# jweyn/DLWP-CS

Hardware: AMD Instinct MI355X
Metric: cubed-sphere samples/sec (fwd+bwd) (higher is better)
Workload: dtype bf16; 1 GPU; unet2 C48: x (32,6,48,48,14) per GPU, 14 out channels, base 32, MSE + Adam, fwd+bwd+update, bf16 activations + bf16 MFMA, fp32 master weights / gradients / Adam; global_batch=32, parallelism=dp1, hip_graphs=True

## Files before the change

dlwp-cs_amd/DLWP/_native.py:

```python
import ctypes
import os
import threading

import numpy as np
import torch

_HERE = os.path.dirname(os.path.abspath(__file__))
_TAG = os.environ.get('DLWPCS_LIB_TAG', '')
LIB_PATH = os.path.join(os.path.dirname(_HERE), 'lib', 'libdlwpcs%s.so' % ('_' + _TAG if _TAG else ''))

F32 = 0
BF16 = 1
MSE_TARGET_F32 = 0x100
MSE_OVERWRITE = 0x200
ADAM_ZERO_GRAD = 1
HEAD_DEFER_STAGE2 = 2
LOSS_MSE, LOSS_MAE, LOSS_ACC = 0, 1, 2
REG_NONE, REG_MSE, REG_MAE, REG_GLOBAL = 0, 1, 2, 3
ACT_NONE = 0
ACT_LEAKY_CLIP = 1
CONV_ACCUMULATE_WGRAD = 1
CONV_PREPACKED = 2
CONV_REUSE_DZ = 4
CONV_DEFER_REDUCE = 8
# ... 118 lines not shown
    'dlwpcs_wgrad_batch_apply': (c_int, [c_void_p, c_int, c_void_p, c_void_p, c_void_p, c_void_p, c_void_p, c_void_p, c_size_t,
                                         c_void_p, c_void_p, c_void_p, c_void_p, c_void_p]),
    'dlwpcs_gconv_fwd': (c_int, [ctypes.POINTER(GConvDesc)] + [c_void_p] * 9),
    'dlwpcs_gconv_bwd_data': (c_int, [ctypes.POINTER(GConvDesc)] + [c_void_p] * 6),
    'dlwpcs_gconv_bwd_weights': (c_int, [ctypes.POINTER(GConvDesc)] + [c_void_p] * 9),
    'dlwpcs_act_fwd': (c_int, [c_void_p, c_void_p, c_size_t, c_int, c_float, c_float, c_int, c_void_p]),
    'dlwpcs_act_bwd': (c_int, [c_void_p, c_void_p, c_void_p, c_size_t, c_int, c_float, c_float, c_int, c_void_p]),
    'dlwpcs_avgpool2_fwd': (c_int, [c_void_p, c_void_p, c_int, c_int, c_int, c_int, c_void_p]),
    'dlwpcs_avgpool2_bwd': (c_int, [c_void_p, c_void_p, c_int, c_int, c_int, c_int, c_void_p]),
    'dlwpcs_avgpool2_bwd_add': (c_int, [c_void_p, c_void_p, c_void_p, c_int, c_int, c_int, c_int, c_void_p]),
    'dlwpcs_avgpool2_bwd_masked': (c_int, [c_void_p, c_void_p, c_void_p, c_void_p, c_int, c_int, c_int, c_float, c_float, c_int,
                                           c_void_p]),
    'dlwpcs_avgpool2_bwd_ring': (c_int, [c_void_p, c_void_p, c_void_p, c_void_p, c_int, c_int, c_int, c_float, c_float, c_int,
                                         c_void_p, c_void_p, c_int, c_int, c_void_p]),
    'dlwpcs_conv_ring_info': (c_int, [ctypes.POINTER(ConvDesc), ctypes.POINTER(c_size_t), ctypes.POINTER(c_int)]),
    'dlwpcs_upsample2_fwd': (c_int, [c_void_p, c_void_p, c_int, c_int, c_int, c_int, c_void_p]),
    'dlwpcs_upsample2_bwd': (c_int, [c_void_p, c_void_p, c_int, c_int, c_int, c_int, c_void_p]),
    'dlwpcs_concat2': (c_int, [c_void_p, c_void_p, c_void_p, c_size_t, c_int, c_int, c_int, c_void_p]),
    'dlwpcs_split2': (c_int, [c_void_p, c_void_p, c_void_p, c_size_t, c_int, c_int, c_int, c_void_p]),
    'dlwpcs_cf_to_cl': (c_int, [c_void_p, c_void_p, c_int, c_int, c_size_t, c_int, c_void_p]),
    'dlwpcs_cl_to_cf': (c_int, [c_void_p, c_void_p, c_int, c_int, c_size_t, c_int, c_void_p]),
    'dlwpcs_add': (c_int, [c_void_p, c_void_p, c_void_p, c_size_t, c_int, c_void_p]),
    'dlwpcs_l1l2_regularize': (c_int, [c_void_p, c_void_p, c_size_t, c_float, c_float, c_float, c_void_p, c_void_p]),
    'dlwpcs_weight_constraint': (c_int, [c_void_p, c_int, c_int, c_int, c_float, c_float, c_float, c_void_p]),
    'dlwpcs_mse_scratch_bytes': (c_size_t, []),
    'dlwpcs_mse_fwd_bwd': (c_int, [c_void_p, c_void_p, c_void_p, c_void_p, c_size_t, c_float, c_int, c_void_p,
                                   c_void_p]),
    'dlwpcs_loss_scratch_bytes': (c_size_t, []),
    'dlwpcs_loss_fwd_bwd': (c_int, [c_void_p, c_void_p, c_void_p, c_void_p, c_void_p, c_size_t, c_int, c_void_p, c_void_p]),
    'dlwpcs_head_loss_step': (c_int, [c_void_p, c_void_p, c_void_p, c_void_p, c_void_p, c_void_p, c_void_p, c_void_p, c_void_p,
# ... 26 lines not shown
    'dlwpcs_batch_gather': (c_int, [c_void_p, ctypes.c_int64, c_int, ctypes.c_int64, c_void_p, c_int, c_void_p, c_int,
                                    c_int, c_int, c_int, c_void_p, c_int, c_int, c_int, c_int, c_int, c_void_p]),
    'dlwpcs_solar_fill': (c_int, [c_void_p, ctypes.c_int64, c_void_p, ctypes.c_int64, c_void_p, c_int, c_int, c_int, c_int,
                                  c_void_p, c_int, c_int, c_int, c_int, c_int, c_void_p]),
    'dlwpcs_comm_load': (c_int, [ctypes.c_char_p]),
    'dlwpcs_comm_unique_id': (c_int, [c_void_p]),
    'dlwpcs_comm_init': (c_int, [ctypes.POINTER(c_void_p), c_void_p, c_int, c_int]),
    'dlwpcs_comm_destroy': (c_int, [c_void_p]),
    'dlwpcs_allreduce_f32': (c_int, [c_void_p, c_void_p, c_size_t, c_void_p]),
    'dlwpcs_lds_oob_probe': (c_int, [c_void_p, c_void_p]),
    'dlwpcs_prof_enable': (c_int, [c_int]),
    'dlwpcs_prof_reset': (c_int, []),
    'dlwpcs_prof_count': (c_int, []),
    'dlwpcs_prof_get': (c_int, [c_int, ctypes.c_char_p, c_int, ctypes.POINTER(ctypes.c_double),
                                ctypes.POINTER(ctypes.c_double), ctypes.POINTER(ctypes.c_double)]),
    'dlwpcs_prof_known_tags': (c_int, []),
    'dlwpcs_prof_known_tag': (c_int, [c_int, ctypes.c_char_p, c_int]),
}

_lib = None
_lock = threading.Lock()


class NativeError(RuntimeError):
    pass


def lib():
    global _lib
    if _lib is None:
# ... 130 lines not shown
```

dlwp-cs_amd/csrc/common.h:

```cpp
#pragma once
#include <hip/hip_runtime.h>
#include <stdint.h>
#include <stdio.h>
#include <stdarg.h>
#include <string.h>
#include "../../include/dlwpcs.h"

namespace dlwpcs {

void set_error(const char *fmt, ...);
int fail(int code, const char *fmt, ...);
const char *last_error();

inline int check_launch(const char *what) {
    hipError_t e = hipGetLastError();
    if (e != hipSuccess) return fail(DLWPCS_E_LAUNCH, "%s: %s", what, hipGetErrorString(e));
    return DLWPCS_OK;
}

bool prof_enabled();
int prof_begin(const char *tag, double flops, double bytes, hipStream_t s);
void prof_end(int idx, hipStream_t s);
int prof_register_tag(const char *tag);
template <typename T> struct KTagType { static const char *str() { return nullptr; } };
template <> struct KTagType<float> { static const char *str() { return "float"; } };
template <> struct KTagType<unsigned short> { static const char *str() { return "unsigned short"; } };
template <typename Name, typename T, auto... Vs> struct KTag {
    static void fmt(char *&p, char *end, bool v) { p += snprintf(p, end - p, "%s", v ? "true" : "false"); }
    static void fmt(char *&p, char *end, int v) { p += snprintf(p, end - p, "%d", v); }
    static const char *str() {
        static char buf[200];
        if (!buf[0]) {
            char *p = buf, *end = buf + sizeof(buf);
            p += snprintf(p, end - p, "%s<", Name::str());
            bool first = true;
            if (KTagType<T>::str()) { p += snprintf(p, end - p, "%s", KTagType<T>::str()); first = false; }
            ((p += snprintf(p, end - p, "%s", first ? "" : ", "), fmt(p, end, Vs), first = false), ...);
// ... 141 lines not shown
```

dlwp-cs_amd/csrc/conv_launch.h:

```cpp
#pragma once
#include "conv_ws.h"

namespace dlwpcs {

struct Work { double flops, bytes; };

static int tile_pixels(int BM, int No) {
    const int face_pix = No * No;
    int pix = BM < face_pix ? BM : face_pix;
    if (No <= BM) {
        int whole = (BM / No) * No;
        if (whole > face_pix) whole = face_pix;
        if (ceil_div(face_pix, whole) <= ceil_div(face_pix, pix)) pix = whole;
    }
    return pix;
}

static long ilv_cost(int pix, int face_pix, int B, int gx, int WM, int *gb, int *fb, bool split, int c2 = 2) {
    auto cost = [&](int npix) { const int mn = (npix + 31) / 32; return 4 * ceil_div(mn, WM) + c2; };
    const int nbl = ceil_div(face_pix, pix), cF = cost(pix), cL = cost(face_pix - (nbl - 1) * pix);
    const long ntiles = 6l * B * nbl;
    const long plain = (long)ceil_div((int)ntiles, gx) * cF;
    if (gb) *gb = 0;
    if (fb) *fb = 0;
    if (!split || cL >= cF || nbl < 2) return plain;
    const long F = 6l * (nbl - 1) * B, S = 6l * B;
    long best = plain;
    for (int GB = 1; GB < gx; ++GB) {
        const int GA = gx - GB;
        const long sB = ceil_div((int)S, GB) * (long)cL;
        for (long mB = 0; mB <= ceil_div((int)F, gx) + 1; ++mB) {
            const long FB = mB * GB < F ? mB * GB : F, FA = F - FB;
            const long cA = (long)ceil_div((int)FA, GA) * cF, cB = mB * cF + sB;
            const long mx = cA > cB ? cA : cB;
            if (mx < best) { best = mx; if (gb) *gb = GB; if (fb) *fb = (int)FB; }
        }
    }
    return best;
}

extern thread_local ConvEdgeArgs g_edge_args;

struct ConvWsName { static const char *str() { return "conv_mfma_ws_kernel"; } };

template <typename T, int KS, int KC, int MT, int NT, int WM, int WN, int VW, int MODE, bool MASK, bool TAIL8 = false, bool MOUT = false,
          bool EDGE = false>
static int launch_conv_cfg(ConvKParams P, const Work &W, hipStream_t s) {
    constexpr int ES = sizeof(T), CGW = 32 / ES;
    constexpr int BM = 32 * MT * WM, NTB = NT * WN, NTHREADS = 64 * WM * WN;
    const int face_pix = P.No * P.No;
    P.ncol = 1;
    if (MODE == MODE_HALO && !EDGE && KS == 3 && (tune_bits() & TUNE_CONV_STRIPS) && P.No >= 64 && P.No % 2 == 0 && P.Cout % (16 / ES) == 0) {
        const int wt = P.No / 2, rows2 = BM / wt, rows1 = BM / P.No;
        if (BM % wt == 0 && rows2 <= P.No && P.No % rows2 == 0 && rows1 >= 1 && rows2 >= 2 * rows1) P.ncol = 2;
    }
    P.Wt = P.No / P.ncol;
// ... 35 lines not shown
    bool pool = MODE != MODE_ZERO && P.pool_out != nullptr && P.No % 2 == 0 && P.Wt % 2 == 0 && (rowpairs || halfrows) &&
                strip_pix % pix == 0 && P.Cout % 32 == 0 && P.Cout % (16 / ES) == 0;
    if (EDGE) pool = pool && !MOUT && ES == 2 && P.dsplit > 0 && P.dsplit % 32 == 0;
    const size_t buf = in_b + w_b;
    size_t patch_b = (size_t)(WM * WN) * 32 * (32 * ES + 16);
    if (pool && 2 * buf + patch_b * MT <= 160 * 1024) patch_b *= MT; else pool = false;
    size_t lds = 2 * buf + patch_b;
    P.patches = 1;
    P.wstat = 0;
    const int nchunks = ceil_div(P.CG, KC / CGW);
    if (nchunks > 2 && nchunks <= 4 && (tune_bits() & TUNE_CONV_WSTAT) && 2 * in_b + nchunks * w_b + patch_b <= 160 * 1024) {
        P.wstat = nchunks;
        lds = 2 * in_b + nchunks * w_b + patch_b;
    } else if (lds > 160 * 1024) { lds = 2 * buf; P.patches = 0; pool = false; }
    if (!pool) P.pool_out = nullptr;
    {
        const bool head = P.head_w != nullptr && P.head_out != nullptr && ES == 2 && NT == 1 && WN == 1 && !EDGE && !MOUT && !MASK &&
                          MODE != MODE_ZERO && P.Cout == 32 && P.patches && !pool;
        if (head) P.out = P.head_out; else P.head_w = nullptr;
        if (P.head_done) *P.head_done = head ? 1 : 0;
    }
    P.colsplit = (pool && halfrows) ? 1 : 0;
    if (P.pool_done) *P.pool_done = pool ? 1 : 0;
    if ((MODE == MODE_ZERO || EDGE) && KS == 3 && P.patches && P.Cout % (16 / ES) == 0 && P.dsplit % (16 / ES) == 0) {
        if (P.direct_done) *P.direct_done = (P.d0 || P.d1) ? 1 : 0;
    } else {
        P.d0 = P.d1 = nullptr;
    }
    if (EDGE) {
        if (P.nblk_face < 2)
// ... 7 lines not shown
        return fail(DLWPCS_E_UNSUPPORTED, "conv: %d tile rows exceed the producers' 5-bit row field", P.tile_rows_max);
    if ((size_t)P.tile_rows_max * P.W2 > (size_t)3 * NTHREADS)
        return fail(DLWPCS_E_UNSUPPORTED, "conv: tile of %d x %d pixels exceeds the producers' register capacity", P.tile_rows_max, P.W2);
    if ((long)6 * face_pix * P.Cout * ES >= (1l << 31))
        return fail(DLWPCS_E_UNSUPPORTED, "conv: one sample of the output (%ld bytes) exceeds the 32-bit store offsets",
                    (long)6 * face_pix * P.Cout * ES);
    if ((long)P.Nin * P.Nin * 6 >= (1l << 16) * 6 && (long)P.Nin * P.Nin >= (1l << 16))
        return fail(DLWPCS_E_UNSUPPORTED, "conv: face size %d too large for the 16-bit index arithmetic", P.Nin);
    auto kern = conv_mfma_ws_kernel<T, KS, KC, MT, NT, WM, WN, VW, MODE, MASK, TAIL8, MOUT, EDGE>;
    if (!MOUT || !(P.d0 || P.d1)) {
        if (!(P.d0)) P.m0 = nullptr;
        if (!(P.d1)) P.m1 = nullptr;
        if (!MOUT) P.m0 = P.m1 = nullptr;
    }
    if (P.mask_done) *P.mask_done = (MOUT && (P.m0 || P.m1)) ? ((P.m0 ? 1 : 0) | (P.m1 ? 2 : 0)) : 0;
    if (lds > 64 * 1024) {
        hipError_t e = hipFuncSetAttribute((const void *)kern, hipFuncAttributeMaxDynamicSharedMemorySize, (int)lds);
        if (e != hipSuccess) return fail(DLWPCS_E_LAUNCH, "conv: hipFuncSetAttribute: %s", hipGetErrorString(e));
    }
    const int gy = ceil_div(P.NTtot, NTB);
    int gx = 256 / gy;
    if (gx < 1) gx = 1;
    if (gx > P.ntiles) gx = P.ntiles;
    dim3 grid((unsigned)gx, (unsigned)gy);
    if (MODE == MODE_ZERO && MT == 3 && sizeof(T) == 4 && (P.tune & TUNE_CONV_ILV) && P.nblk_face > 1 && gx > 1)
        (void)ilv_cost(pix, face_pix, P.B, gx, WM, &P.split_gb, &P.split_fb, true);
    if (P.ilv_fwd) { P.split_gb = fwd_gb; P.split_fb = fwd_fb; }
    if (P.dry_run) return DLWPCS_OK;
    int pidx = -1;
    const char *tag = KTag<ConvWsName, T, KS, KC, MT, NT, WM, WN, VW, MODE, MASK, TAIL8, MOUT, EDGE>::tag();
    if (prof_enabled()) {
        pidx = prof_begin(tag, W.flops, W.bytes, s);
    }
    hipLaunchKernelGGL(kern, grid, dim3(2 * NTHREADS), lds, s, P, g_edge_args);
    if (pidx >= 0) prof_end(pidx, s);
    return check_launch("conv_mfma");
}

template <typename T, int KS, int VW, int MODE, bool MASK, bool MOUT = false, bool EDGE = false>
static int launch_conv(const ConvKParams &P, const Work &W, hipStream_t s) {
    const int face_pix = P.No * P.No;
    constexpr int VWF = 16 / (int)sizeof(T);
    constexpr int K2 = 64 / (int)sizeof(T);
    constexpr int K1 = K2 / 2;
    if constexpr (KS == 1) return launch_conv_cfg<T, KS, K1, 3, 1, 4, 1, VW, MODE, MASK, false, MOUT, EDGE>(P, W, s);
    else if constexpr (VW != VWF) return launch_conv_cfg<T, KS, K1, 3, 1, 4, 1, VW, MODE, MASK, false, MOUT, EDGE>(P, W, s);
    else {
// ... 35 lines not shown
```

dlwp-cs_amd/csrc/conv_mfma.hip:

```cpp
#include <stdlib.h>
#include <type_traits>
#include "common.h"
#include "mfma_common.h"
#include "conv_ws.h"
#include "conv_launch.h"

namespace dlwpcs {

template <typename T>
__device__ __forceinline__ void pack_weights_range(const float *__restrict__ w_eq, const float *__restrict__ w_pol,
                                                   const float *__restrict__ w_np, T *__restrict__ out,
                                                   int KS, int Cin, int Cout, int K, int Ncol, int CG, int NTtot,
                                                   int flip, int transposed, size_t total, size_t first, size_t stride) {
    constexpr int J = 16 / (int)sizeof(T);
    const int TAPS = KS * KS;
    const size_t entries = total / J;
    for (size_t e = first; e < entries; e += stride) {
        unsigned r = (unsigned)e;
        const int n = r % 32; r /= 32;
        const int hf = r % 2; r /= 2;
        const int tap = r % TAPS; r /= TAPS;
        const int cg = r % CG; r /= CG;
        const int nt = r % NTtot; r /= NTtot;
        const int v = (int)r;
// ... 1108 lines not shown
}

static bool pw_applies(const dlwpcs_conv_desc *d) {
    return d->dtype == DLWPCS_BF16 && d->ksize == 1 && !d->halo && !d->up0 && d->C1 == 0 && d->C0 == 32 && d->Cout % 2 == 0 &&
           d->Cout >= 8 && d->Cout <= 32 && ((long)d->N * d->N) % 16 == 0 && d->B > 0 &&
           (long)d->B * 6 * d->N * d->N * 32 < (1l << 31);
}
static unsigned pw_grid(long ngroups) {
    long blocks = (ngroups + 4 * PW_U - 1) / (4 * PW_U);
    return (unsigned)(blocks > 2048 ? 2048 : blocks);
}

static inline int cin_logical(const dlwpcs_conv_desc *d);

thread_local ConvEdgeArgs g_edge_args{};

struct WgradBf16Name { static const char *str() { return "wgrad_bf16_kernel"; } };
struct WgradMfmaName { static const char *str() { return "wgrad_mfma_kernel"; } };
struct PwHeadName { static const char *str() { return "pw_head_train_kernel"; } };
struct PwFwdName { static const char *str() { return "pw_fwd_kernel"; } };
static const int g_plain_tags[] = {prof_register_tag("pw_dgrad_kernel<false>"), prof_register_tag("pw_dgrad_kernel<true>"),
                                   prof_register_tag("wgrad_reduce_batch_kernel")};

static int dispatch_conv(int dtype, int KS, int vw, const ConvKParams &P, const Work &W, hipStream_t s) {
    if (KS == 3 && P.mode == MODE_HALO && P.edge) {
        if (dtype == DLWPCS_BF16 && vw == 8) return dispatch_conv_edge(P, W, s);
        return fail(DLWPCS_E_UNSUPPORTED, "conv: gather-form data gradient serves bf16 with 16-B channel vectors");
    }
    return dtype == DLWPCS_BF16 ? dispatch_conv_bf16(KS, vw, P, W, s) : dispatch_conv_f32(KS, vw, P, W, s);
}
// ... 390 lines not shown
    const int NTtot = ceil_div(d->Cout, 32);
    if (b_eq && !prepacked) {
        const int n = 3 * NTtot * 32;
        hipLaunchKernelGGL(pack_bias_kernel, dim3(ceil_div(n, 256)), dim3(256), 0, s, (const float *)b_eq,
                           (const float *)b_pol, (const float *)b_np, (float *)(ws + L.bias), d->Cout, NTtot * 32);
    }
    ConvKParams P{};
    P.src0 = src0; P.src1 = src1; P.ymask = nullptr;
    P.wpk = wpk; P.bias = b_eq ? bpk : nullptr; P.out = y; P.table = table_dev;
    P.B = d->B; P.Nin = d->N; P.No = out_size(d);
    P.C0 = d->C0; P.C1 = d->C1; P.Cin = Cin; P.Cout = d->Cout;
    P.CG = ceil_div(Cin, cgw_of(d->dtype)); P.NTtot = NTtot; P.up0 = d->up0;
    P.mode = d->halo ? MODE_HALO : MODE_DIRECT;
    P.act = d->act; P.alpha = d->alpha; P.vmax = d->vmax;
    P.pool_out = y_pooled; P.pool_done = pool_done;
    if (head) { P.head_w = head->wpk; P.head_b = head->bias; P.head_out = head->out; P.head_done = head->done; }
    if ((d->flags & DLWPCS_CONV_OUT_PADDED) && !pw_applies(d))
        return fail(DLWPCS_E_UNSUPPORTED, "conv_fwd: DLWPCS_CONV_OUT_PADDED serves the bf16 pointwise output layer only");
    if (pw_applies(d)) {
        PwParams Q{};
        Q.in = (const bf16_t *)src0; Q.wpk = (const bf16_t *)wpk; Q.bias = b_eq ? bpk : nullptr; Q.out = (bf16_t *)y;
        Q.ngroups = (long)d->B * 6 * d->N * d->N / 16; Q.groups_per_face = d->N * d->N / 16; Q.Cout = d->Cout;
        if (d->flags & DLWPCS_CONV_OUT_PADDED) Q.Cout = (d->Cout + 7) / 8 * 8;
        Q.alpha = d->alpha; Q.vmax = d->vmax;
        int pidx = -1;
        const bool actv = d->act != DLWPCS_ACT_NONE;
        if (prof_enabled()) {
            const Work wk = conv_work(d);
            const char *tag = Q.Cout <= 16 ? (actv ? KTag<PwFwdName, void, true, 1>::tag() : KTag<PwFwdName, void, false, 1>::tag())
                                           : (actv ? KTag<PwFwdName, void, true, 2>::tag() : KTag<PwFwdName, void, false, 2>::tag());
// ... 4 lines not shown
            if (actv) hipLaunchKernelGGL((pw_fwd_kernel<true, 1>), pgrid, dim3(256), 0, s, Q);
            else hipLaunchKernelGGL((pw_fwd_kernel<false, 1>), pgrid, dim3(256), 0, s, Q);
        } else {
            if (actv) hipLaunchKernelGGL((pw_fwd_kernel<true, 2>), pgrid, dim3(256), 0, s, Q);
            else hipLaunchKernelGGL((pw_fwd_kernel<false, 2>), pgrid, dim3(256), 0, s, Q);
        }
        if (pidx >= 0) prof_end(pidx, s);
        return check_launch("pw_fwd");
    }
    if (d->dtype == DLWPCS_BF16 && d->ksize == 3 && d->halo && d->C1 == 0 && d->C0 >= 8 && d->C0 % 2 == 0 && d->C0 % 8 != 0 &&
        NTtot <= 2) {
        return dispatch_conv_tail8(d->C0 <= 16 ? 16 : 32, NTtot, P, conv_work(d), s);
    }
    return dispatch_conv(d->dtype, d->ksize, vec_width(d->C0, d->C1, d->dtype), P, conv_work(d), s);
}

static int conv_bwd_data_impl(const dlwpcs_conv_desc *d, const void *dy, const void *y, bool dz_given,
                              const void *w_eq, const void *w_pol, const void *w_np,
                              void *dsrc0, void *dsrc1, const void *m0, const void *m1, float m_alpha, float m_vmax,
                              const int32_t *inv_table_dev, void *workspace, size_t workspace_bytes, dlwpcs_stream_t stream,
                              const char *who, int *ring_query = nullptr) {
    int rc = validate(d, who);
    if (rc) return rc;
    const bool prepacked = (d->flags & DLWPCS_CONV_PREPACKED) != 0;
    if (!dy || !w_eq || (!w_pol && !prepacked) || !workspace) return fail(DLWPCS_E_INVALID, "%s: null pointer", who);
    const bool has_act = d->act != DLWPCS_ACT_NONE && !dz_given;
    if (has_act && !y) return fail(DLWPCS_E_INVALID, "%s: activation needs the saved output y", who);
    if (d->halo && !inv_table_dev) return fail(DLWPCS_E_INVALID, "%s: halo requested without inverse table", who);
    if ((m0 || m1) && (!(m_alpha >= 0.f) || !(m_vmax >= 0.f)))
        return fail(DLWPCS_E_INVALID, "%s: mask activation needs negative_slope >= 0 and max_value >= 0, got %g / %g", who, m_alpha, m_vmax);
// ... 162 lines not shown
    if (!d->halo || d->ksize != 3 || d->up0 || d->B < 1) return 0;
    const WsLayout L = ws_layout(d);
    int q = 0;
    char dummy = 0;
    dlwpcs_conv_desc dd = *d;
    dd.act = DLWPCS_ACT_NONE;
    dd.flags |= DLWPCS_CONV_PREPACKED;
    const int rc = conv_bwd_data_impl(&dd, &dummy, nullptr, true, &dummy, nullptr, nullptr, &dummy, d->C1 > 0 ? &dummy : nullptr, nullptr,
                                      nullptr, 0.f, 0.f, (const int32_t *)&dummy, &dummy, L.total, nullptr, "conv_ring_info", &q);
    if (rc || !q) return 0;
    *dxv_offset = L.dxv;
    *channels = d->C0 + d->C1;
    return 1;
}

extern "C" int dlwpcs_conv_bwd_weights(const dlwpcs_conv_desc *d, const void *src0, const void *src1, const void *dy,
                                       const void *y, void *dw_eq, void *dw_pol, void *dw_np,
                                       void *db_eq, void *db_pol, void *db_np, const int32_t *table_dev,
                                       void *workspace, size_t workspace_bytes, dlwpcs_stream_t stream) {
    int rc = validate(d, "conv_bwd_weights");
    if (rc) return rc;
    if (!src0 || !dy || !dw_eq || !dw_pol || !workspace) return fail(DLWPCS_E_INVALID, "conv_bwd_weights: null pointer");
    if (d->C1 > 0 && !src1) return fail(DLWPCS_E_INVALID, "conv_bwd_weights: C1 > 0 but src1 is null");
    if (d->act != DLWPCS_ACT_NONE && !y) return fail(DLWPCS_E_INVALID, "conv_bwd_weights: activation needs the saved output y");
    if (d->halo && !table_dev) return fail(DLWPCS_E_INVALID, "conv_bwd_weights: halo requested without table");
    if ((db_np != nullptr) != (dw_np != nullptr) && db_eq) return fail(DLWPCS_E_INVALID, "conv_bwd_weights: dw_np/db_np must match");
    const WsLayout L = ws_layout(d);
    if (workspace_bytes < L.total) return fail(DLWPCS_E_WORKSPACE, "conv_bwd_weights: workspace %zu < %zu bytes", workspace_bytes, L.total);
    hipStream_t s = (hipStream_t)stream;
    char *ws = (char *)workspace;
// ... 195 lines not shown
```

dlwp-cs_amd/csrc/conv_ws.h:

```cpp
#pragma once
#include <stdlib.h>
#include <type_traits>
#include "common.h"
#include "mfma_common.h"

namespace dlwpcs {

enum { MODE_DIRECT = 0, MODE_HALO = 1, MODE_ZERO = 2 };

struct ConvKParams {
    const void *src0, *src1;
    const void *ymask;
    const void *wpk;
    const float *bias;
    void *out;
    const int32_t *table;
    int edge;
    int B, Nin, No;
    int C0, C1, Cin, Cout;
    int CG, NTtot;
    int up0;
    int mode;
    int act;
    float alpha, vmax;
// ... 21 lines not shown
    void *head_out;
    int *head_done;
    int tune;
    int tile_rows_max;
    int ntiles;
    int split_gb, split_fb;
    int Wt, ncol;
    uint32_t magicWt, magicNcol;
    int ilv_fwd;
};

struct ConvEdgeArgs { const int32_t *src; int8_t wids[36]; };

enum { TUNE_WG_PRODUCER_PRIO = 1, TUNE_CONV_PRODUCER_PRIO = 2, TUNE_CONV_WEIGHTS_STAY = 4, TUNE_CONV_SPLIT_N = 16,
       TUNE_CONV_SPLIT2_BWD = 32, TUNE_CONV_WSTAT = 64, TUNE_CONV_STAGGER = 256, TUNE_CONV_ILV = 512, TUNE_CONV_STRIPS = 1024,
       TUNE_CONV_ILV_FWD = 2048 };
static int tune_bits() {
    static int v = -1;
    if (v < 0) { const char *e = getenv("DLWPCS_TUNE"); v = e ? atoi(e) : (TUNE_WG_PRODUCER_PRIO | TUNE_CONV_PRODUCER_PRIO | TUNE_CONV_WEIGHTS_STAY | TUNE_CONV_SPLIT_N | TUNE_CONV_SPLIT2_BWD | TUNE_CONV_WSTAT |
                               TUNE_CONV_STAGGER | TUNE_CONV_ILV | TUNE_CONV_STRIPS | TUNE_CONV_ILV_FWD | (3 << 12));
                 }
    return v;
}

template <typename T, int KS, int KC, int MT, int NT, int WM, int WN, int VW, int MODE, bool MASK, bool TAIL8 = false, bool MOUT = false,
          bool EDGE = false>
__device__ __forceinline__ void conv_ws_body(const ConvKParams &P, char *smem, const uint32_t lw, const int G, const int by,
                                             const ConvEdgeArgs &E = ConvEdgeArgs{}) {
    static_assert(!TAIL8 || (VW == 8 && sizeof(T) == 2 && !MASK), "TAIL8: bf16 16-B vectors, forward only");
    static_assert(!MOUT || ((MODE == MODE_ZERO || EDGE) && KS == 3 && sizeof(T) == 2 && !MASK), "MOUT: bf16 data gradient, direct mode");
    static_assert(!EDGE || (MODE == MODE_HALO && KS == 3 && !MASK && !TAIL8 && VW * sizeof(T) == 16), "EDGE: gather-form data gradient");
// ... 18 lines not shown
    typedef typename VecT<T, VW>::type V;
    const int in_bytes = P.tile_rows_max * P.W2 * RB;
    const int in_step = P.wstat ? in_bytes : in_bytes + WF4 * 16;
    const int w_base = P.wstat ? 2 * in_bytes : in_bytes;
    const int w_step = P.wstat ? WF4 * 16 : in_bytes + WF4 * 16;
    const int patch_base = P.wstat ? 2 * in_bytes + P.wstat * WF4 * 16 : 2 * (in_bytes + WF4 * 16);

    const int tid = threadIdx.x;
    const bool is_producer = tid >= NCT;
    const int nt0 = by * NTB;
    const int face_pix = P.No * P.No;
    const int strip_pix = P.No * P.Wt;
    const int g0 = P.up0 ? (P.Nin >> 1) : P.Nin;
    const int nchunks = (P.CG + KCG - 1) / KCG;

    constexpr bool ILV_OK = (MODE == MODE_ZERO || (MODE == MODE_HALO && !EDGE && KS == 3)) && MT == 3 && sizeof(T) == 4;
    const bool ilv = ILV_OK && (P.tune & TUNE_CONV_ILV) != 0 && (MODE == MODE_ZERO || P.ilv_fwd != 0);
    const int nbl = P.nblk_face;
    const bool csplit = ilv && P.split_gb > 0;
    int t_first = 0, t_last = 0;
    int f0 = 0, f1 = 0, s0 = 0, s1 = 0;
    if (csplit) {
        const int GB = P.split_gb, GA = G - GB;
        const int Ftot = 6 * (nbl - 1) * P.B, Stot = 6 * P.B, FA = Ftot - P.split_fb;
        if ((int)lw < GA) {
            f0 = (int)(((long)FA * lw) / GA); f1 = (int)(((long)FA * (lw + 1)) / GA);
        } else {
            const int u = (int)lw - GA;
            f0 = FA + (int)(((long)P.split_fb * u) / GB); f1 = FA + (int)(((long)P.split_fb * (u + 1)) / GB);
            s0 = (int)(((long)Stot * u) / GB); s1 = (int)(((long)Stot * (u + 1)) / GB);
        }
    } else {
        t_first = (int)(((long)P.ntiles * lw) / G);
        t_last = (int)(((long)P.ntiles * (lw + 1)) / G);
    }
    const int n_my = csplit ? (f1 - f0) + (s1 - s0) : t_last - t_first;
    auto tile_of = [&](int q) __attribute__((always_inline)) {
        if (!csplit) return t_first + q;
        const int nf = f1 - f0, perF = (nbl - 1) * P.B;
        if (q < nf) { const int i = f0 + q, f = i / perF; return f * nbl * P.B + (i - f * perF); }
        const int i = s0 + (q - nf), f = i / P.B;
        return f * nbl * P.B + perF + (i - f * P.B);
    };
    if ((P.tune & TUNE_CONV_STAGGER) && !csplit && n_my * G < P.ntiles) {
#pragma unroll 1
// ... 670 lines not shown
        load_frag(0, fa[0], fb[0]);
        __builtin_amdgcn_sched_group_barrier(0x100, MTA + NT, 0);
#pragma unroll
        for (int step = 0; step < NSTEP; ++step) {
            const int cur = step & 1;
            if (step + 1 < NSTEP) load_frag(step + 1, fa[cur ^ 1], fb[cur ^ 1]);
#pragma unroll
            for (int mt = 0; mt < MTA; ++mt)
#pragma unroll
                for (int nt = 0; nt < NT; ++nt) frag_mma<T>(acc[mt][nt], fb[cur][nt], fa[cur][mt]);
            __builtin_amdgcn_sched_group_barrier(0x100, MTA + NT, 0);
            __builtin_amdgcn_sched_group_barrier(0x008, MmaPerFrag<T>::N * MTA * NT, 0);
        }
    };

    auto mma_chunk_edge = [&](const Geo &gq, int ch, auto two_tag) {
      if constexpr (EDGE) {
        constexpr int NSETS = decltype(two_tag)::value ? 2 : 1;
        constexpr int NX = NSETS * 3 * KCG;
        const char *lds_in = smem + (g & 1) * in_step, *lds_w = smem + w_base + (P.wstat ? ch : (g & 1)) * w_step;
        const char *lds_x = lds_w + WF4M * 16;
        uint32_t (&rs)[MT][3] = es;
        uint32_t (&rw)[(MT + 3) / 4] = ewp;
#pragma unroll
        for (int mt = 0; mt < MT; ++mt) asm volatile("" : "+v"(rs[mt][0]), "+v"(rs[mt][1]), "+v"(rs[mt][2]));
#pragma unroll
        for (int w = 0; w < (MT + 3) / 4; ++w) asm volatile("" : "+v"(rw[w]));
        uint4 fa[2][MT], fb[2][NT];
        auto load_frag = [&](int step, uint4 (&a)[MT], uint4 (&bw)[NT]) {
            if (step < NSTEP) {
                const int cgl = step / TAPS, tap = step % TAPS;
                const int dy = tap / KS, dx = tap % KS;
                const int tapoff = (dy * P.W2 + dx) * RB + cgl * 32;
#pragma unroll
                for (int mt = 0; mt < MT; ++mt) {
                    int base = abase[mt];
                    if (tap != TAPS / 2) base += (int)((rw[mt / 4] >> (8 * (mt % 4) + (tap < TAPS / 2 ? tap : tap - 1))) & 1u) << 23;
                    a[mt] = *reinterpret_cast<const uint4 *>(lds_in + base + tapoff);
                }
#pragma unroll
                for (int nt = 0; nt < NT; ++nt)
                    bw[nt] = *reinterpret_cast<const uint4 *>(
                        lds_w + ((((wn * NT + nt) * KCG + cgl) * TAPS + tap) * 2 + half) * 512 + l31 * 16);
            } else {
                const int x = step - NSTEP, j = x / KCG, cgl = x % KCG;
#pragma unroll
                for (int mt = 0; mt < MT; ++mt) {
                    const uint32_t f16 = (j & 1) ? rs[mt][j >> 1] >> 16 : rs[mt][j >> 1] & 0xffffu;
                    a[mt] = *reinterpret_cast<const uint4 *>(lds_in + (int)(f16 << 4) + cgl * 32);
                }
#pragma unroll
                for (int nt = 0; nt < NT; ++nt)
                    bw[nt] = *reinterpret_cast<const uint4 *>(
                        lds_x + (((j % 3) * NTB * KCG + (wn * NT + nt) * KCG + cgl) * 2 + half) * 512 + l31 * 16);
            }
        };
        load_frag(0, fa[0], fb[0]);
        __builtin_amdgcn_sched_group_barrier(0x100, MT + NT, 0);
#pragma unroll
        for (int step = 0; step < NSTEP + NX; ++step) {
            const int cur = step & 1;
            if (step + 1 < NSTEP + NX) load_frag(step + 1, fa[cur ^ 1], fb[cur ^ 1]);
#pragma unroll
            for (int mt = 0; mt < MT; ++mt)
#pragma unroll
                for (int nt = 0; nt < NT; ++nt) frag_mma<T>(acc[mt][nt], fb[cur][nt], fa[cur][mt]);
            __builtin_amdgcn_sched_group_barrier(0x100, MT + NT, 0);
            __builtin_amdgcn_sched_group_barrier(0x008, MmaPerFrag<T>::N * MT * NT, 0);
        }
      }
    };

    const bool lines = P.patches && (P.Cout % (16 / ES)) == 0;
    for (int q = 0; q < n_my; ++q) {
        const Geo gq = geo_of(tile_of(q));
        setup(gq);
        mask_load(gq);
        pool_mask_load(gq);
        const int my_mt = ilv ? max(0, min(MT, (((gq.npix + 31) >> 5) - wm + WM - 1) / WM)) : MT;
        for (int ch = 0; ch < nchunks; ++ch, ++g) {
            asm volatile("s_waitcnt lgkmcnt(0)" ::: "memory");
            __builtin_amdgcn_s_barrier();
            if constexpr (ILV_OK) {
                if (my_mt >= MT) mma_chunk(ch, std::integral_constant<int, MT>{});
                else if (my_mt == 2) mma_chunk(ch, std::integral_constant<int, 2>{});
                else if (my_mt == 1) mma_chunk(ch, std::integral_constant<int, 1>{});
            } else if constexpr (EDGE) {
                if (!e_any) mma_chunk(ch, std::integral_constant<int, MT>{});
                else if (!e_two) mma_chunk_edge(gq, ch, std::false_type{});
                else mma_chunk_edge(gq, ch, std::true_type{});
            } else {
                mma_chunk(ch, std::integral_constant<int, MT>{});
            }
        }
        if constexpr (HEAD_OK) {
            if (headed) {
                if (fast_act) head_apply(std::integral_constant<int, 1>{});
                else head_apply(std::integral_constant<int, 0>{});
            }
        }
        if (lines) {
            if constexpr (ILV_OK) {
                if (my_mt >= MT) epilogue_lines(gq, acc, std::integral_constant<int, MT>{});
                else if (my_mt == 2) epilogue_lines(gq, acc, std::integral_constant<int, 2>{});
                else if (my_mt == 1) epilogue_lines(gq, acc, std::integral_constant<int, 1>{});
// ... 19 lines not shown
```

dlwp-cs_amd/csrc/prof.cpp:

```cpp
#include <mutex>
#include <string>
#include <vector>
#include <stdio.h>
#include <string.h>
#include "common.h"

namespace dlwpcs {

struct ProfRecord {
    std::string tag;
    double flops, bytes;
    hipEvent_t e0, e1;
};

static std::mutex g_mu;
static bool g_enabled = false;
static std::vector<ProfRecord> g_records;

bool prof_enabled() { return g_enabled; }

static std::vector<std::string> &known_tags() { static std::vector<std::string> v; return v; }
int prof_register_tag(const char *tag) {
    auto &v = known_tags();
    for (size_t i = 0; i < v.size(); ++i) if (v[i] == tag) return (int)i;
    v.push_back(tag);
// ... 39 lines not shown
    std::lock_guard<std::mutex> lk(g_mu);
    ProfRecord r;
    r.tag = tag; r.flops = flops; r.bytes = bytes;
    if (capturing(s)) r.tag += "@graph";
    if (hipEventCreate(&r.e0) != hipSuccess || hipEventCreate(&r.e1) != hipSuccess) return -1;
    record(r.e0, s);
    g_records.push_back(r);
    return (int)g_records.size() - 1;
}

void prof_end(int idx, hipStream_t s) {
    std::lock_guard<std::mutex> lk(g_mu);
    if (idx >= 0 && idx < (int)g_records.size()) record(g_records[idx].e1, s);
}

}

using namespace dlwpcs;

extern "C" int dlwpcs_prof_enable(int on) {
    std::lock_guard<std::mutex> lk(g_mu);
    g_enabled = on != 0;
    return DLWPCS_OK;
}

extern "C" int dlwpcs_prof_reset(void) {
    std::lock_guard<std::mutex> lk(g_mu);
    for (auto &r : g_records) { (void)hipEventDestroy(r.e0); (void)hipEventDestroy(r.e1); }
    g_records.clear();
    return DLWPCS_OK;
// ... 6 lines not shown

extern "C" int dlwpcs_prof_get(int i, char *tag, int tag_len, double *ms, double *flops, double *bytes) {
    std::lock_guard<std::mutex> lk(g_mu);
    if (i < 0 || i >= (int)g_records.size() || !tag || tag_len < 1 || !ms || !flops || !bytes)
        return fail(DLWPCS_E_INVALID, "prof_get: bad arguments");
    ProfRecord &r = g_records[i];
    if (hipEventSynchronize(r.e1) != hipSuccess) return fail(DLWPCS_E_LAUNCH, "prof_get: event sync failed");
    float t = 0.f;
    if (hipEventElapsedTime(&t, r.e0, r.e1) != hipSuccess) return fail(DLWPCS_E_LAUNCH, "prof_get: elapsed time failed");
    strncpy(tag, r.tag.c_str(), tag_len - 1);
    tag[tag_len - 1] = 0;
    *ms = t; *flops = r.flops; *bytes = r.bytes;
    return DLWPCS_OK;
}

extern "C" int dlwpcs_prof_known_tags(void) { return (int)known_tags().size(); }

extern "C" int dlwpcs_prof_known_tag(int i, char *tag, int tag_len) {
    const auto &v = known_tags();
    if (i < 0 || i >= (int)v.size() || !tag || tag_len < 1) return fail(DLWPCS_E_INVALID, "prof_known_tag: bad arguments");
    strncpy(tag, v[i].c_str(), tag_len - 1);
    tag[tag_len - 1] = 0;
    return DLWPCS_OK;
}
```

include/dlwpcs.h:

```cpp
#ifndef DLWPCS_H
#define DLWPCS_H

#include <stddef.h>
#include <stdint.h>

#ifdef __cplusplus
extern "C" {
#endif

#define DLWPCS_VERSION 105

#define DLWPCS_OK             0
#define DLWPCS_E_INVALID     -1
#define DLWPCS_E_UNSUPPORTED -2
#define DLWPCS_E_WORKSPACE   -3
#define DLWPCS_E_LAUNCH      -4

#define DLWPCS_F32  0
#define DLWPCS_BF16 1

#define DLWPCS_ACT_NONE        0
#define DLWPCS_ACT_LEAKY_CLIP  1

typedef void *dlwpcs_stream_t;
// ... 299 lines not shown
                        const int32_t *var_idx_dev, int nv, int n_steps, int t_off, int t_stride, void *out,
                        int Ctot, int c_off, int c_stride, int channels_last, int dtype, dlwpcs_stream_t stream);

int dlwpcs_solar_fill(const double *row_tab, int64_t T, const double *cell_tab, int64_t S, const int32_t *samples_dev, int B,
                      int n_steps, int t_off, int t_stride, void *out, int Ctot, int c_off, int c_stride, int channels_last,
                      int dtype, dlwpcs_stream_t stream);

int dlwpcs_comm_load(const char *librccl_path);
int dlwpcs_comm_unique_id(void *id128);
int dlwpcs_comm_init(void **comm, const void *id128, int rank, int world);
int dlwpcs_comm_destroy(void *comm);
int dlwpcs_allreduce_f32(void *comm, float *buf, size_t n, dlwpcs_stream_t stream);

int dlwpcs_lds_oob_probe(int32_t *nonzero_dev, dlwpcs_stream_t stream);

int dlwpcs_prof_enable(int on);
int dlwpcs_prof_reset(void);
int dlwpcs_prof_count(void);
int dlwpcs_prof_get(int i, char *tag, int tag_len, double *ms, double *flops, double *bytes);
int dlwpcs_prof_known_tags(void);
int dlwpcs_prof_known_tag(int i, char *tag, int tag_len);

#ifdef __cplusplus
}
#endif
#endif
```

Measured before the change: 47940 samples/s.

## Extend interleaved partial-tile scheduling to bf16 conv and add plan/profile introspection

Lets the bf16 3x3 conv kernels (forward halo and dgrad, including edge-gather) run partial last tiles with fewer M-tiles and spread tile work across workgroups through a mixed full/last-tile split with reversed ordering. This is meant to cut wasted MFMA work on ragged face tiles and even out the load per workgroup. The new path is gated by tune bits that are not in the visible default mask. It also adds a dry-run plan query API and per-launch profiling detail strings.

```diff
diff --git a/dlwp-cs_amd/DLWP/_native.py b/dlwp-cs_amd/DLWP/_native.py
--- a/dlwp-cs_amd/DLWP/_native.py
+++ b/dlwp-cs_amd/DLWP/_native.py
@@ -156,6 +156,7 @@
     'dlwpcs_avgpool2_bwd_ring': (c_int, [c_void_p, c_void_p, c_void_p, c_void_p, c_int, c_int, c_int, c_float, c_float, c_int,
                                          c_void_p, c_void_p, c_int, c_int, c_void_p]),
     'dlwpcs_conv_ring_info': (c_int, [ctypes.POINTER(ConvDesc), ctypes.POINTER(c_size_t), ctypes.POINTER(c_int)]),
+    'dlwpcs_conv_plan': (c_int, [ctypes.POINTER(ConvDesc), c_int, ctypes.POINTER(ctypes.c_int32)]),
     'dlwpcs_upsample2_fwd': (c_int, [c_void_p, c_void_p, c_int, c_int, c_int, c_int, c_void_p]),
     'dlwpcs_upsample2_bwd': (c_int, [c_void_p, c_void_p, c_int, c_int, c_int, c_int, c_void_p]),
     'dlwpcs_concat2': (c_int, [c_void_p, c_void_p, c_void_p, c_size_t, c_int, c_int, c_int, c_void_p]),
@@ -212,6 +213,7 @@
     'dlwpcs_prof_count': (c_int, []),
     'dlwpcs_prof_get': (c_int, [c_int, ctypes.c_char_p, c_int, ctypes.POINTER(ctypes.c_double),
                                 ctypes.POINTER(ctypes.c_double), ctypes.POINTER(ctypes.c_double)]),
+    'dlwpcs_prof_get_detail': (c_int, [c_int, ctypes.c_char_p, c_int]),
     'dlwpcs_prof_known_tags': (c_int, []),
     'dlwpcs_prof_known_tag': (c_int, [c_int, ctypes.c_char_p, c_int]),
 }
diff --git a/dlwp-cs_amd/csrc/common.h b/dlwp-cs_amd/csrc/common.h
--- a/dlwp-cs_amd/csrc/common.h
+++ b/dlwp-cs_amd/csrc/common.h
@@ -21,6 +21,7 @@
 bool prof_enabled();
 int prof_begin(const char *tag, double flops, double bytes, hipStream_t s);
 void prof_end(int idx, hipStream_t s);
+void prof_detail(int idx, const char *text);
 int prof_register_tag(const char *tag);
 template <typename T> struct KTagType { static const char *str() { return nullptr; } };
 template <> struct KTagType<float> { static const char *str() { return "float"; } };
diff --git a/dlwp-cs_amd/csrc/conv_launch.h b/dlwp-cs_amd/csrc/conv_launch.h
--- a/dlwp-cs_amd/csrc/conv_launch.h
+++ b/dlwp-cs_amd/csrc/conv_launch.h
@@ -16,7 +16,7 @@
     return pix;
 }
 
-static long ilv_cost(int pix, int face_pix, int B, int gx, int WM, int *gb, int *fb, bool split, int c2 = 2) {
+static long ilv_cost(int pix, int face_pix, int B, int gx, int WM, int *gb, int *fb, bool split, int c2 = 2, bool mixed = false) {
     auto cost = [&](int npix) { const int mn = (npix + 31) / 32; return 4 * ceil_div(mn, WM) + c2; };
     const int nbl = ceil_div(face_pix, pix), cF = cost(pix), cL = cost(face_pix - (nbl - 1) * pix);
     const long ntiles = 6l * B * nbl;
@@ -36,10 +36,20 @@
             if (mx < best) { best = mx; if (gb) *gb = GB; if (fb) *fb = (int)FB; }
         }
     }
+    if (mixed) {
+        long mx = 0;
+        for (int w = 0; w < gx; ++w) {
+            const int u = gx - 1 - w;
+            const long c = (F * (w + 1) / gx - F * w / gx) * cF + (S * (u + 1) / gx - S * u / gx) * cL;
+            if (c > mx) mx = c;
+        }
+        if (mx < best) { best = mx; if (gb) *gb = gx; if (fb) *fb = (int)F; }
+    }
     return best;
 }
 
 extern thread_local ConvEdgeArgs g_edge_args;
+extern thread_local int32_t *g_plan_out;
 
 struct ConvWsName { static const char *str() { return "conv_mfma_ws_kernel"; } };
 
@@ -105,6 +115,12 @@
         lds = 2 * in_b + nchunks * w_b + patch_b;
     } else if (lds > 160 * 1024) { lds = 2 * buf; P.patches = 0; pool = false; }
     if (!pool) P.pool_out = nullptr;
+    bool ilv_bf16 = false;
+    if ((MODE == MODE_ZERO || MODE == MODE_HALO) && KS == 3 && MT == 3 && sizeof(T) == 2 && !TAIL8 && VW == 8 && WM > 1 &&
+        (tune_bits() & (EDGE ? TUNE_CONV_ILV_EDGE : TUNE_CONV_ILV_BF16)) && P.ncol == 1 && !pool && face_pix <= 1024) {
+        const int last = face_pix - (ceil_div(face_pix, pix) - 1) * pix;
+        if (ceil_div(ceil_div(last, 32), WM) < MT) { ilv_bf16 = true; P.ilv_fwd = 1; }
+    }
     {
         const bool head = P.head_w != nullptr && P.head_out != nullptr && ES == 2 && NT == 1 && WN == 1 && !EDGE && !MOUT && !MASK &&
                           MODE != MODE_ZERO && P.Cout == 32 && P.patches && !pool;
@@ -142,7 +158,7 @@
         if (!MOUT) P.m0 = P.m1 = nullptr;
     }
     if (P.mask_done) *P.mask_done = (MOUT && (P.m0 || P.m1)) ? ((P.m0 ? 1 : 0) | (P.m1 ? 2 : 0)) : 0;
-    if (lds > 64 * 1024) {
+    if (lds > 64 * 1024 && !P.dry_run) {
         hipError_t e = hipFuncSetAttribute((const void *)kern, hipFuncAttributeMaxDynamicSharedMemorySize, (int)lds);
         if (e != hipSuccess) return fail(DLWPCS_E_LAUNCH, "conv: hipFuncSetAttribute: %s", hipGetErrorString(e));
     }
@@ -154,11 +170,27 @@
     if (MODE == MODE_ZERO && MT == 3 && sizeof(T) == 4 && (P.tune & TUNE_CONV_ILV) && P.nblk_face > 1 && gx > 1)
         (void)ilv_cost(pix, face_pix, P.B, gx, WM, &P.split_gb, &P.split_fb, true);
     if (P.ilv_fwd) { P.split_gb = fwd_gb; P.split_fb = fwd_fb; }
+    if (ilv_bf16 && P.nblk_face > 1 && gx > 1) (void)ilv_cost(pix, face_pix, P.B, gx, WM, &P.split_gb, &P.split_fb, true, 2, true);
+    if (g_plan_out) {
+        const int32_t v[10] = {pix, P.nblk_face, P.ntiles, gx, gy, MT, WM, P.ilv_fwd, P.split_gb, P.split_fb};
+        for (int i = 0; i < 10; ++i) g_plan_out[i] = v[i];
+    }
     if (P.dry_run) return DLWPCS_OK;
     int pidx = -1;
     const char *tag = KTag<ConvWsName, T, KS, KC, MT, NT, WM, WN, VW, MODE, MASK, TAIL8, MOUT, EDGE>::tag();
     if (prof_enabled()) {
         pidx = prof_begin(tag, W.flops, W.bytes, s);
+        long charged = 0;
+        for (int t = 0; t < P.nblk_face; ++t) {
+            const int np = strip_pix - t * pix < pix ? strip_pix - t * pix : pix;
+            charged += 32l * WM * (P.ilv_fwd || (ES == 4 && MODE == MODE_ZERO && MT == 3 && (P.tune & TUNE_CONV_ILV)) ? ceil_div(ceil_div(np, 32), WM) : MT);
+        }
+        char det[256];
+        snprintf(det, sizeof det, "B=%d N=%d No=%d C0=%d C1=%d Cout=%d up0=%d %s grid=%dx%d tiles=%d tiles_per_wg=%.2f tile_pix=%d chunks=%d held=%ld charged=%ld "
+                 "ilv=%d split=%d/%d wstat=%d pool=%d", P.B, P.Nin, P.No, P.C0, P.C1, P.Cout, P.up0,
+                 EDGE ? "dgrad_gather" : (MODE == MODE_ZERO ? "dgrad_padded" : "fwd"), gx, gy, P.ntiles, (double)P.ntiles / gx, pix, nchunks,
+                 6l * P.B * face_pix, 6l * P.B * P.ncol * charged, P.ilv_fwd, P.split_gb, P.split_fb, P.wstat, P.pool_out ? 1 : 0);
+        prof_detail(pidx, det);
     }
     hipLaunchKernelGGL(kern, grid, dim3(2 * NTHREADS), lds, s, P, g_edge_args);
     if (pidx >= 0) prof_end(pidx, s);
diff --git a/dlwp-cs_amd/csrc/conv_mfma.hip b/dlwp-cs_amd/csrc/conv_mfma.hip
--- a/dlwp-cs_amd/csrc/conv_mfma.hip
+++ b/dlwp-cs_amd/csrc/conv_mfma.hip
@@ -1146,6 +1146,7 @@
 static inline int cin_logical(const dlwpcs_conv_desc *d);
 
 thread_local ConvEdgeArgs g_edge_args{};
+thread_local int32_t *g_plan_out = nullptr;
 
 struct WgradBf16Name { static const char *str() { return "wgrad_bf16_kernel"; } };
 struct WgradMfmaName { static const char *str() { return "wgrad_mfma_kernel"; } };
@@ -1566,6 +1567,7 @@
     P.mode = d->halo ? MODE_HALO : MODE_DIRECT;
     P.act = d->act; P.alpha = d->alpha; P.vmax = d->vmax;
     P.pool_out = y_pooled; P.pool_done = pool_done;
+    P.dry_run = g_plan_out ? 1 : 0;
     if (head) { P.head_w = head->wpk; P.head_b = head->bias; P.head_out = head->out; P.head_done = head->done; }
     if ((d->flags & DLWPCS_CONV_OUT_PADDED) && !pw_applies(d))
         return fail(DLWPCS_E_UNSUPPORTED, "conv_fwd: DLWPCS_CONV_OUT_PADDED serves the bf16 pointwise output layer only");
@@ -1600,6 +1602,7 @@
     }
     return dispatch_conv(d->dtype, d->ksize, vec_width(d->C0, d->C1, d->dtype), P, conv_work(d), s);
 }
+
 
 static int conv_bwd_data_impl(const dlwpcs_conv_desc *d, const void *dy, const void *y, bool dz_given,
                               const void *w_eq, const void *w_pol, const void *w_np,
@@ -1792,6 +1795,29 @@
     return 1;
 }
 
+extern "C" int dlwpcs_conv_plan(const dlwpcs_conv_desc *d, int pass, int32_t *plan10) {
+    int rc = validate(d, "conv_plan");
+    if (rc) return rc;
+    if (!plan10 || d->ksize != 3 || d->B < 1 || (pass != 0 && pass != 1)) return fail(DLWPCS_E_INVALID, "conv_plan: 3 x 3 layers, pass 0 or 1");
+    for (int i = 0; i < 10; ++i) plan10[i] = 0;
+    char dummy = 0;
+    dlwpcs_conv_desc dd = *d;
+    dd.flags |= DLWPCS_CONV_PREPACKED;
+    const WsLayout L = ws_layout(&dd);
+    g_plan_out = plan10;
+    if (pass == 0) {
+        rc = conv_fwd_impl(&dd, &dummy, d->C1 > 0 ? &dummy : nullptr, &dummy, nullptr, nullptr, &dummy, nullptr, nullptr, &dummy,
+                           (const int32_t *)&dummy, &dummy, L.total, nullptr, nullptr, nullptr, nullptr);
+    } else {
+        int q = 0;
+        dd.act = DLWPCS_ACT_NONE;
+        rc = conv_bwd_data_impl(&dd, &dummy, nullptr, true, &dummy, nullptr, nullptr, &dummy, d->C1 > 0 ? &dummy : nullptr, nullptr, nullptr,
+                                0.f, 0.f, (const int32_t *)&dummy, &dummy, L.total, nullptr, "conv_plan", &q);
+    }
+    g_plan_out = nullptr;
+    return rc;
+}
+
 extern "C" int dlwpcs_conv_bwd_weights(const dlwpcs_conv_desc *d, const void *src0, const void *src1, const void *dy,
                                        const void *y, void *dw_eq, void *dw_pol, void *dw_np,
                                        void *db_eq, void *db_pol, void *db_np, const int32_t *table_dev,
diff --git a/dlwp-cs_amd/csrc/conv_ws.h b/dlwp-cs_amd/csrc/conv_ws.h
--- a/dlwp-cs_amd/csrc/conv_ws.h
+++ b/dlwp-cs_amd/csrc/conv_ws.h
@@ -59,7 +59,7 @@
 
 enum { TUNE_WG_PRODUCER_PRIO = 1, TUNE_CONV_PRODUCER_PRIO = 2, TUNE_CONV_WEIGHTS_STAY = 4, TUNE_CONV_SPLIT_N = 16,
        TUNE_CONV_SPLIT2_BWD = 32, TUNE_CONV_WSTAT = 64, TUNE_CONV_STAGGER = 256, TUNE_CONV_ILV = 512, TUNE_CONV_STRIPS = 1024,
-       TUNE_CONV_ILV_FWD = 2048 };
+       TUNE_CONV_ILV_FWD = 2048, TUNE_CONV_ILV_BF16 = 1 << 18, TUNE_CONV_ILV_EDGE = 1 << 19 };
 static int tune_bits() {
     static int v = -1;
     if (v < 0) { const char *e = getenv("DLWPCS_TUNE"); v = e ? atoi(e) : (TUNE_WG_PRODUCER_PRIO | TUNE_CONV_PRODUCER_PRIO | TUNE_CONV_WEIGHTS_STAY | TUNE_CONV_SPLIT_N | TUNE_CONV_SPLIT2_BWD | TUNE_CONV_WSTAT |
@@ -108,8 +108,9 @@
     const int g0 = P.up0 ? (P.Nin >> 1) : P.Nin;
     const int nchunks = (P.CG + KCG - 1) / KCG;
 
-    constexpr bool ILV_OK = (MODE == MODE_ZERO || (MODE == MODE_HALO && !EDGE && KS == 3)) && MT == 3 && sizeof(T) == 4;
-    const bool ilv = ILV_OK && (P.tune & TUNE_CONV_ILV) != 0 && (MODE == MODE_ZERO || P.ilv_fwd != 0);
+    constexpr bool ILV_OK = (MODE == MODE_ZERO || (MODE == MODE_HALO && KS == 3)) && MT == 3 && KS == 3 &&
+                            (sizeof(T) == 4 || (!TAIL8 && VW == 8 && WM > 1));
+    const bool ilv = ILV_OK && (sizeof(T) == 4 ? (P.tune & TUNE_CONV_ILV) != 0 && (MODE == MODE_ZERO || P.ilv_fwd != 0) : P.ilv_fwd != 0);
     const int nbl = P.nblk_face;
     const bool csplit = ilv && P.split_gb > 0;
     int t_first = 0, t_last = 0;
@@ -122,7 +123,8 @@
         } else {
             const int u = (int)lw - GA;
             f0 = FA + (int)(((long)P.split_fb * u) / GB); f1 = FA + (int)(((long)P.split_fb * (u + 1)) / GB);
-            s0 = (int)(((long)Stot * u) / GB); s1 = (int)(((long)Stot * (u + 1)) / GB);
+            const int us = GA == 0 ? GB - 1 - u : u;
+            s0 = (int)(((long)Stot * us) / GB); s1 = (int)(((long)Stot * (us + 1)) / GB);
         }
     } else {
         t_first = (int)(((long)P.ntiles * lw) / G);
@@ -823,8 +825,9 @@
         }
     };
 
-    auto mma_chunk_edge = [&](const Geo &gq, int ch, auto two_tag) {
+    auto mma_chunk_edge = [&](const Geo &gq, int ch, auto two_tag, auto mta_tag) {
       if constexpr (EDGE) {
+        constexpr int MTA = decltype(mta_tag)::value;
         constexpr int NSETS = decltype(two_tag)::value ? 2 : 1;
         constexpr int NX = NSETS * 3 * KCG;
         const char *lds_in = smem + (g & 1) * in_step, *lds_w = smem + w_base + (P.wstat ? ch : (g & 1)) * w_step;
@@ -832,7 +835,7 @@
         uint32_t (&rs)[MT][3] = es;
         uint32_t (&rw)[(MT + 3) / 4] = ewp;
 #pragma unroll
-        for (int mt = 0; mt < MT; ++mt) asm volatile("" : "+v"(rs[mt][0]), "+v"(rs[mt][1]), "+v"(rs[mt][2]));
+        for (int mt = 0; mt < MTA; ++mt) asm volatile("" : "+v"(rs[mt][0]), "+v"(rs[mt][1]), "+v"(rs[mt][2]));
 #pragma unroll
         for (int w = 0; w < (MT + 3) / 4; ++w) asm volatile("" : "+v"(rw[w]));
         uint4 fa[2][MT], fb[2][NT];
@@ -842,7 +845,7 @@
                 const int dy = tap / KS, dx = tap % KS;
                 const int tapoff = (dy * P.W2 + dx) * RB + cgl * 32;
 #pragma unroll
-                for (int mt = 0; mt < MT; ++mt) {
+                for (int mt = 0; mt < MTA; ++mt) {
                     int base = abase[mt];
                     if (tap != TAPS / 2) base += (int)((rw[mt / 4] >> (8 * (mt % 4) + (tap < TAPS / 2 ? tap : tap - 1))) & 1u) << 23;
                     a[mt] = *reinterpret_cast<const uint4 *>(lds_in + base + tapoff);
@@ -854,7 +857,7 @@
             } else {
                 const int x = step - NSTEP, j = x / KCG, cgl = x % KCG;
 #pragma unroll
-                for (int mt = 0; mt < MT; ++mt) {
+                for (int mt = 0; mt < MTA; ++mt) {
                     const uint32_t f16 = (j & 1) ? rs[mt][j >> 1] >> 16 : rs[mt][j >> 1] & 0xffffu;
                     a[mt] = *reinterpret_cast<const uint4 *>(lds_in + (int)(f16 << 4) + cgl * 32);
                 }
@@ -865,17 +868,17 @@
             }
         };
         load_frag(0, fa[0], fb[0]);
-        __builtin_amdgcn_sched_group_barrier(0x100, MT + NT, 0);
+        __builtin_amdgcn_sched_group_barrier(0x100, MTA + NT, 0);
 #pragma unroll
         for (int step = 0; step < NSTEP + NX; ++step) {
             const int cur = step & 1;
             if (step + 1 < NSTEP + NX) load_frag(step + 1, fa[cur ^ 1], fb[cur ^ 1]);
 #pragma unroll
-            for (int mt = 0; mt < MT; ++mt)
+            for (int mt = 0; mt < MTA; ++mt)
 #pragma unroll
                 for (int nt = 0; nt < NT; ++nt) frag_mma<T>(acc[mt][nt], fb[cur][nt], fa[cur][mt]);
-            __builtin_amdgcn_sched_group_barrier(0x100, MT + NT, 0);
-            __builtin_amdgcn_sched_group_barrier(0x008, MmaPerFrag<T>::N * MT * NT, 0);
+            __builtin_amdgcn_sched_group_barrier(0x100, MTA + NT, 0);
+            __builtin_amdgcn_sched_group_barrier(0x008, MmaPerFrag<T>::N * MTA * NT, 0);
         }
       }
     };
@@ -890,14 +893,21 @@
         for (int ch = 0; ch < nchunks; ++ch, ++g) {
             asm volatile("s_waitcnt lgkmcnt(0)" ::: "memory");
             __builtin_amdgcn_s_barrier();
+            auto chunk = [&](auto mta_tag) __attribute__((always_inline)) {
+                if constexpr (EDGE) {
+                    if (!e_any) mma_chunk(ch, mta_tag);
+                    else if (!e_two) mma_chunk_edge(gq, ch, std::false_type{}, mta_tag);
+                    else mma_chunk_edge(gq, ch, std::true_type{}, mta_tag);
+                } else {
+                    mma_chunk(ch, mta_tag);
+                }
+            };
             if constexpr (ILV_OK) {
-                if (my_mt >= MT) mma_chunk(ch, std::integral_constant<int, MT>{});
-                else if (my_mt == 2) mma_chunk(ch, std::integral_constant<int, 2>{});
-                else if (my_mt == 1) mma_chunk(ch, std::integral_constant<int, 1>{});
+                if (my_mt >= MT) chunk(std::integral_constant<int, MT>{});
+                else if (my_mt == 2) chunk(std::integral_constant<int, 2>{});
+                else if (my_mt == 1) chunk(std::integral_constant<int, 1>{});
             } else if constexpr (EDGE) {
-                if (!e_any) mma_chunk(ch, std::integral_constant<int, MT>{});
-                else if (!e_two) mma_chunk_edge(gq, ch, std::false_type{});
-                else mma_chunk_edge(gq, ch, std::true_type{});
+                chunk(std::integral_constant<int, MT>{});
             } else {
                 mma_chunk(ch, std::integral_constant<int, MT>{});
             }
diff --git a/dlwp-cs_amd/csrc/prof.cpp b/dlwp-cs_amd/csrc/prof.cpp
--- a/dlwp-cs_amd/csrc/prof.cpp
+++ b/dlwp-cs_amd/csrc/prof.cpp
@@ -8,7 +8,7 @@
 namespace dlwpcs {
 
 struct ProfRecord {
-    std::string tag;
+    std::string tag, detail;
     double flops, bytes;
     hipEvent_t e0, e1;
 };
@@ -78,6 +78,11 @@
     if (idx >= 0 && idx < (int)g_records.size()) record(g_records[idx].e1, s);
 }
 
+void prof_detail(int idx, const char *text) {
+    std::lock_guard<std::mutex> lk(g_mu);
+    if (idx >= 0 && idx < (int)g_records.size() && text) g_records[idx].detail = text;
+}
+
 }
 
 using namespace dlwpcs;
@@ -114,6 +119,14 @@
     return DLWPCS_OK;
 }
 
+extern "C" int dlwpcs_prof_get_detail(int i, char *text, int text_len) {
+    std::lock_guard<std::mutex> lk(g_mu);
+    if (i < 0 || i >= (int)g_records.size() || !text || text_len < 1) return fail(DLWPCS_E_INVALID, "prof_get_detail: bad arguments");
+    strncpy(text, g_records[i].detail.c_str(), text_len - 1);
+    text[text_len - 1] = 0;
+    return DLWPCS_OK;
+}
+
 extern "C" int dlwpcs_prof_known_tags(void) { return (int)known_tags().size(); }
 
 extern "C" int dlwpcs_prof_known_tag(int i, char *tag, int tag_len) {
diff --git a/include/dlwpcs.h b/include/dlwpcs.h
--- a/include/dlwpcs.h
+++ b/include/dlwpcs.h
@@ -337,10 +337,13 @@
 
 int dlwpcs_lds_oob_probe(int32_t *nonzero_dev, dlwpcs_stream_t stream);
 
+int dlwpcs_conv_plan(const dlwpcs_conv_desc *d, int pass, int32_t *plan10);
+
 int dlwpcs_prof_enable(int on);
 int dlwpcs_prof_reset(void);
 int dlwpcs_prof_count(void);
 int dlwpcs_prof_get(int i, char *tag, int tag_len, double *ms, double *flops, double *bytes);
+int dlwpcs_prof_get_detail(int i, char *text, int text_len);
 int dlwpcs_prof_known_tags(void);
 int dlwpcs_prof_known_tag(int i, char *tag, int tag_len);
 
```

After: 46200 samples/s. -3.6%, worse.
